# terryye/cuda_FlashAttention

Measured on AMD Instinct MI355X. Metric: FA2 fwd+bwd TFLOP/s at (B=4,H=16,N=8192,d=128); % MFMA peak, higher is better.
Workload: dtype bf16; 1 GPU; FA2 forward+backward bf16, (B=4,H=16,N=8192,d=128) per GPU, non-causal (BASELINE configs[2]); flops = 14 B H N^2 d; B=4, H=16, N=8192, d=128, parallelism=head-sharded replicas x1

## Files before the change

### cuda_flashattention_amd/csrc/fa2_bwd_bf16.hip

```cpp
#include <type_traits>

#include "fa2_regfile.h"
#include "fa2_launch.h"

namespace fa2 {

constexpr float kNoKeyRC = -1.0e30f;
constexpr float kNoKeyLq = 1.0e30f;

template <int D>
__global__ void __launch_bounds__(256) fa2_bwd_delta_kernel(const __bf16* __restrict__ dO,
                                                            const __bf16* __restrict__ O,
                                                            const float* __restrict__ L, const float* __restrict__ dL,
                                                            float* __restrict__ Dv, float* __restrict__ RC,
                                                            size_t rows, int nq, int q_hs, int q_row0, size_t rc_plane,
                                                            float inv_scale)
{
    const size_t r = ((size_t)blockIdx.x * 256 + threadIdx.x) >> 4;
    const int sub = threadIdx.x & 15;
    const size_t head = r / (size_t)nq, i = r % (size_t)nq;
    const size_t row = head * (size_t)q_hs + i;
    const size_t prow = row + (size_t)q_row0;
    float acc = 0.0f;
    if (r < rows) {
#pragma unroll
        for (int c = sub * 8; c < D; c += 128) {
            const bf16x8 a = *reinterpret_cast<const bf16x8*>(dO + row * D + c);
            const bf16x8 b = *reinterpret_cast<const bf16x8*>(O + row * D + c);
#pragma unroll
            for (int e = 0; e < 8; ++e) acc += (float)a[e] * (float)b[e];
        }
    }
#pragma unroll
    for (int off = 8; off >= 1; off >>= 1) acc += __shfl_xor(acc, off, 16);
    if (r < rows && sub == 0) {
        const float l = L[row];
        if (dL) {
            const float g = dL[row];
            acc -= l == -INFINITY ? 0.0f : g;
        }
        Dv[prow] = acc;
        RC[prow] = l == -INFINITY ? kNoKeyRC : -l * inv_scale;
        RC[rc_plane + prow] = -acc;
    }
}

__global__ void __launch_bounds__(256) fa2_bwd_dsink_kernel(const float* __restrict__ Dv, const float* __restrict__ L,
                                                            const float* __restrict__ sink, float* __restrict__ dsink,
                                                            int batch, int heads, int nq, int q_hs, int q_row0)
{
// ... 439 lines not shown
            constexpr int dt = decltype(G)::value / 4, g = decltype(G)::value % 4;
            constexpr int RK = A_DK + 16 * (kb * DT + dt) + 4 * g, RV = A_DV + 16 * (kb * DT + dt) + 4 * g;
            bf16x4 a, b;
            a[0] = (__bf16)(aread<RK>() * p.scale); a[1] = (__bf16)(aread<RK + 1>() * p.scale);
            a[2] = (__bf16)(aread<RK + 2>() * p.scale); a[3] = (__bf16)(aread<RK + 3>() * p.scale);
            b[0] = (__bf16)aread<RV>(); b[1] = (__bf16)aread<RV + 1>();
            b[2] = (__bf16)aread<RV + 2>(); b[3] = (__bf16)aread<RV + 3>();
            if (key < N) {
                *reinterpret_cast<bf16x4*>(dKk + 2 * (32 * dt + 8 * g + 4 * h)) = a;
                *reinterpret_cast<bf16x4*>(dVk + 2 * (32 * dt + 8 * g + 4 * h)) = b;
            }
        });
    });
}

template <int D, bool CAUSAL>
__global__ void __launch_bounds__(256, 1) __attribute__((amdgpu_num_vgpr(60))) fa2_bwd_dkdv_kernel(BwdArgs p)
{
    const int ncb = (p.Nk + kDkKeys - 1) / kDkKeys;
    int kvhead, cb;
    map_block(blockIdx.x, p.BH / p.kv_group, ncb, kvhead, cb);
    bwd_dkdv_impl<D, CAUSAL>(p, kvhead, cb);
}

template <int D, bool CAUSAL>
__global__ void __launch_bounds__(256, 1) __attribute__((amdgpu_num_vgpr(60))) fa2_bwd_dkdv_varlen_kernel(VarlenBwdArgs v)
{
    int kvhead, idx;
    map_block(blockIdx.x, v.a.BH / v.a.kv_group, v.n_key_items, kvhead, idx);
    const VarlenItem it = uniform_item(v.key_items, idx);
    bwd_dkdv_impl<D, CAUSAL>(bwd_varlen_view<D>(v.a, it), kvhead, it.block);
}

template <int D, bool CAUSAL>
static hipError_t launch_bwd_one(const BwdArgs& a, hipStream_t stream, const SinkGrad* sg)
{
    const size_t rows = (size_t)a.BH * a.Nq;
    hipError_t e = hipSuccess;
    if (a.phases & 1) {
        hipLaunchKernelGGL((fa2_bwd_delta_kernel<D>), dim3((unsigned)((rows * 16 + 255) / 256)), dim3(256), 0,
                           stream, (const __bf16*)a.dO, (const __bf16*)a.O, a.L, sg ? sg->dL : nullptr, a.D, a.RC, rows, a.Nq, a.q_hs,
                           a.q_row0, (size_t)a.BH * a.q_hs, 1.0f / a.scale);
        e = hipGetLastError();
        if (e != hipSuccess) return e;
        if (sg && sg->sink && (e = launch_dsink(*sg, a, a.Nq, stream)) != hipSuccess) return e;
    }
    const int nb = (a.Nq + kBwdRows - 1) / kBwdRows;
    constexpr int lds_dq = 3 * 2 * kDqKV * D * 2;
    constexpr int lds_dk = kDkKeys * D * 2 + 2 * (2 * 2 * kDkQ * D * 2 + 512);
    if (a.phases & 2) {
        e = launch_lds<fa2_bwd_dq_kernel<D, CAUSAL>>(dim3((unsigned)(nb * a.BH)), dim3(256), lds_dq, stream, a);
        if (e != hipSuccess) return e;
    }
    if (a.phases & 4) {
        const int ncb = (a.Nk + kDkKeys - 1) / kDkKeys;
        e = launch_lds<fa2_bwd_dkdv_kernel<D, CAUSAL>>(dim3((unsigned)(ncb * (a.BH / a.kv_group))), dim3(256), lds_dk, stream, a);
    }
    return e;
}

template <int D, bool CAUSAL>
static hipError_t launch_bwd_varlen_one(const VarlenBwdArgs& v, hipStream_t stream, const SinkGrad* sg)
{
    const BwdArgs& a = v.a;
    const size_t rows = (size_t)a.BH * a.q_hs;
    hipLaunchKernelGGL((fa2_bwd_delta_kernel<D>), dim3((unsigned)((rows * 16 + 255) / 256)), dim3(256), 0, stream,
                       (const __bf16*)a.dO, (const __bf16*)a.O, a.L, sg ? sg->dL : nullptr, a.D, a.RC, rows, a.q_hs, a.q_hs, 0, rows,
                       1.0f / a.scale);
    hipError_t e = hipGetLastError();
    if (e != hipSuccess) return e;
    if (sg && sg->sink && (e = launch_dsink(*sg, a, a.q_hs, stream)) != hipSuccess) return e;
    constexpr int lds_dq = 3 * 2 * kDqKV * D * 2;
    constexpr int lds_dk = kDkKeys * D * 2 + 2 * (2 * 2 * kDkQ * D * 2 + 512);
    e = launch_lds<fa2_bwd_dq_varlen_kernel<D, CAUSAL>>(dim3((unsigned)(v.n_row_items * a.BH)), dim3(256), lds_dq, stream, v);
    if (e != hipSuccess) return e;
    return launch_lds<fa2_bwd_dkdv_varlen_kernel<D, CAUSAL>>(dim3((unsigned)(v.n_key_items * (a.BH / a.kv_group))), dim3(256), lds_dk,
                                                            stream, v);
}

hipError_t launch_bwd_varlen_bf16(const VarlenBwdArgs& v, hipStream_t stream, const SinkGrad* sg)
{
    const BwdArgs& a = v.a;
    if (a.kv_group < 1 || a.BH % a.kv_group != 0 || v.n_row_items < 1 || v.n_key_items < 1 || !v.row_items || !v.key_items)
        return hipErrorInvalidValue;
    if (a.d == 128) return a.causal ? launch_bwd_varlen_one<128, true>(v, stream, sg) : launch_bwd_varlen_one<128, false>(v, stream, sg);
    if (a.d == 64) return a.causal ? launch_bwd_varlen_one<64, true>(v, stream, sg) : launch_bwd_varlen_one<64, false>(v, stream, sg);
    return hipErrorInvalidValue;
}

hipError_t launch_bwd_bf16(const BwdArgs& a, hipStream_t stream, const SinkGrad* sg)
{
    if (a.kv_group < 1 || a.BH % a.kv_group != 0) return hipErrorInvalidValue;
    if (a.d == 128) return a.causal ? launch_bwd_one<128, true>(a, stream, sg) : launch_bwd_one<128, false>(a, stream, sg);
    if (a.d == 64) return a.causal ? launch_bwd_one<64, true>(a, stream, sg) : launch_bwd_one<64, false>(a, stream, sg);
    return hipErrorInvalidValue;
}

}
```

### cuda_flashattention_amd/csrc/fa2_bwd_fused.hip

```cpp
#include <cstdlib>
#include <cstring>
#include <type_traits>

#include "fa2_regfile.h"
#include "fa2_launch.h"

namespace fa2 {

#include "fa2_bwd_fused_body.inc"

typedef __attribute__((address_space(3))) void* fused_lptr_t;

#ifndef FA2_FUSED_DSKEY
#define FA2_FUSED_DSKEY(row) (((row) >> 1) & 7)
#endif

#ifndef FA2_FUSED_DIAG
#define FA2_FUSED_DIAG 0
#endif

constexpr int kFusedRegFile = RF512;

#define FA2_FUSED_CLOBBERS "memory", "vcc", FA2_RF512
#define FA2_FUSED_OPS_128 [r0] "v"(roff[0]), [r1] "v"(roff[1]), [r2] "v"(roff[2]), [r3] "v"(roff[3]), [r4] "v"(roff[4]), [r5] "v"(roff[5]),  \
// ... 50 lines not shown
        "buffer_atomic_add_f32 v%c9, %0, %1, s12 offen offset:1024\n\tbuffer_atomic_add_f32 v%c10, %0, %1, s12 offen offset:1536\n\t"
        "buffer_atomic_add_f32 v%c11, %0, %1, s13 offen\n\tbuffer_atomic_add_f32 v%c12, %0, %1, s13 offen offset:512\n\t"
        "buffer_atomic_add_f32 v%c13, %0, %1, s13 offen offset:1024\n\tbuffer_atomic_add_f32 v%c14, %0, %1, s13 offen offset:1536\n\t"
        "buffer_atomic_add_f32 v%c15, %0, %1, s14 offen\n\tbuffer_atomic_add_f32 v%c16, %0, %1, s14 offen offset:512\n\t"
        "buffer_atomic_add_f32 v%c17, %0, %1, s14 offen offset:1024\n\tbuffer_atomic_add_f32 v%c18, %0, %1, s14 offen offset:1536\n\t"
        "s_nop 1"
        : : "v"(voff), "s"(rs), "s"(soff), "i"(DQT), "i"(DQT + 1), "i"(DQT + 2), "i"(DQT + 3), "i"(DQT + 4), "i"(DQT + 5), "i"(DQT + 6),
            "i"(DQT + 7), "i"(DQT + 8), "i"(DQT + 9), "i"(DQT + 10), "i"(DQT + 11), "i"(DQT + 12), "i"(DQT + 13), "i"(DQT + 14),
            "i"(DQT + 15)
        : "memory", "s12", "s13", "s14", "v255");
}

template <int VF, int KS, int S>
__device__ __forceinline__ void fused_load_vfrag(const char* v0, const char* v1)
{
#ifndef FA2_FUSED_KV_NT
#define FA2_FUSED_KV_NT ""
#define FA2_FUSED_KV_AUX 0
#endif
    asm volatile("global_load_dwordx4 v[%c2:%c3], %0, off offset:%c4" FA2_FUSED_KV_NT "\n\tglobal_load_dwordx4 v[%c5:%c6], %1, off offset:%c4" FA2_FUSED_KV_NT
                 : : "v"(v0), "v"(v1), "i"(VF + 4 * S), "i"(VF + 4 * S + 3), "i"(32 * S), "i"(VF + 4 * (KS + S)), "i"(VF + 4 * (KS + S) + 3)
                 : "memory", "v255");
}

template <int DQT>
__device__ __forceinline__ void fused_dq_zero()
{
    static_for<16>([&](auto R) { vset<kFusedRegFile, CL_TOP, DQT + decltype(R)::value>(0u); });
}

constexpr int kCtlTicket = 0, kCtlNextHead = 32 * 16, kCtlError = 32 * 17, kCtlHeadmap = 32 * 18;
constexpr int kHmPad = 16;
constexpr int kSpinLimit = FA2_FUSED_SPIN_LIMIT;

struct FusedArgs {
    BwdArgs b;
    float* dQacc;
    int* ctl;
    int npad;
    const float* rc;
    int fault;
};

#ifdef FA2_TEST_HOOKS
static int g_hook_fault = 0, g_hook_grid = 0, g_hook_last_grid = 0;
extern "C" void fa2_test_set_fused_hooks(int fault, int grid) { g_hook_fault = fault; g_hook_grid = grid; }
extern "C" int fa2_test_last_fused_grid(void) { return g_hook_last_grid; }
#define FA2_HOOK_NOTE_GRID(n) (g_hook_last_grid = (n))
#else
constexpr int g_hook_fault = 0, g_hook_grid = 0;
#define FA2_HOOK_NOTE_GRID(n) ((void)0)
#endif

__device__ __forceinline__ int fused_ctl_ints(int BH, int ncb) { return kCtlHeadmap + 16 * (BH + kHmPad) + 9 * BH * ncb; }

__device__ __forceinline__ int fused_load_sc1(const int* p)
{
    int v;
    asm volatile("global_load_dword %0, %1, off sc1\n\ts_waitcnt vmcnt(0)" : "=v"(v) : "v"(p) : "memory");
    return v;
}
__device__ __forceinline__ void fused_seen_set(int v)
{
    asm volatile("v_mov_b32 v39, %0" : : "s"(v) : "v39");
}

__device__ __forceinline__ int fused_lane_id() { return (int)__builtin_amdgcn_mbcnt_hi(~0u, __builtin_amdgcn_mbcnt_lo(~0u, 0u)); }
template <int OFF>
__device__ __forceinline__ int fused_mail_read(uint32_t lds_addr)
{
    int v;
    asm volatile("v_mov_b32 %0, %1\n\tds_read_b32 %0, %0 offset:%c2\n\ts_waitcnt lgkmcnt(0)" : "=&v"(v) : "s"(lds_addr), "i"(OFF) : "memory");
    return __builtin_amdgcn_readfirstlane(v);
}

__device__ __forceinline__ void fused_store_flag(int* p, int v)
{
    asm volatile("global_store_dword %0, %1, off" : : "v"(p), "v"(v) : "memory");
}

__device__ __forceinline__ bool fused_spin_over(int* ctl, int spins)
{
    if (spins > kSpinLimit) {
        atomicExch(ctl + kCtlError, 1);
        return true;
    }
    return (spins & 1023) == 0 && fused_load_sc1(ctl + kCtlError) != 0;
}

template <bool CHAIN, bool CAUSAL, bool RAGGED = false, bool RECT = false, int HD = 128>
__global__ void __launch_bounds__(256, 1) __attribute__((amdgpu_num_vgpr(39))) fa2_bwd_fused_kernel(FusedArgs fp)
{
    static_assert(CHAIN || !RAGGED, "the atomics form has no ragged variant");
    static_assert(!RECT || (CHAIN && !CAUSAL && !RAGGED), "rectangular blocks: chained, unmasked, aligned");
    static_assert(HD == 128 || (HD == 64 && CHAIN && !RECT), "head_dim 64: chained, square");
    extern __shared__ __attribute__((aligned(16))) char smem[];
    const BwdArgs& p = fp.b;
    constexpr int D = HD, ROWB = 2 * D, KS = D / 16, DT = D / 32;
    constexpr int DQW = 128;
    constexpr int TROWS = 32;
    constexpr bool W = D == 128;
    constexpr int QRING = W ? FA2_FUSED_QRING : FA2_FUSED64_QRING, BUFB = W ? FA2_FUSED_BUFB : FA2_FUSED64_BUFB,
                  DSB = W ? FA2_FUSED_DSB : FA2_FUSED64_DSB, LDSB = W ? FA2_FUSED_LDS : FA2_FUSED64_LDS;
    constexpr int CPR = D / 8, RPI = 64 / CPR, NINS = TROWS / RPI;
    constexpr int VF = W ? FA2_FUSED_VF : FA2_FUSED64_VF, DQT = W ? FA2_FUSED_DQT : FA2_FUSED64_DQT,
                  ROFFK = W ? FA2_FUSED_ROFFK : FA2_FUSED64_ROFFK, DSWR = W ? FA2_FUSED_DSWR : FA2_FUSED64_DSWR,
                  DSRD = W ? FA2_FUSED_DSRD : FA2_FUSED64_DSRD, KT = W ? FA2_FUSED_KT : FA2_FUSED64_KT;
    constexpr int VMW = CHAIN ? (W ? 4 : 2) : 63;
    int* const mail = reinterpret_cast<int*>(smem + LDSB);
    const uint32_t mail_addr = __builtin_amdgcn_readfirstlane((uint32_t)(uintptr_t)smem) + LDSB;

    const int tid = threadIdx.x;
    const int lane = tid & 63;
    const int wave = __builtin_amdgcn_readfirstlane(tid >> 6);
    const int ki = lane & 31;
    const int h = lane >> 5;
    const int N = p.Nk;
    const int NP = RAGGED ? fp.npad : N;
    const int NQ = RECT ? p.Nq : N;
    const int NPQ = RECT ? NQ : NP;
    const int QHS = RECT ? p.q_hs : N, KHS = RECT ? p.k_hs : N;
    const int QR0 = RECT ? p.q_row0 : 0;
    const int ncb = NP / 256;
    const int ntiles = NPQ / TROWS;
    const int niter = ((ntiles + 1 + 5) / 6) * 6;
    const float c2 = p.scale * kLog2e;
    const size_t rc_plane = (size_t)p.BH * (RECT ? QHS : NP);

    const uint32_t lbase = (uint32_t)(uintptr_t)smem;
    const int trq = (lane & 15) >> 2, trp = lane & 3, trcb = (lane >> 4) & 1;
    uint32_t roff[KS], toff[2 * DT];
#pragma unroll
    for (int s = 0; s < KS; ++s) roff[s] = lbase + QRING + lds_off<D>(ki, 2 * s + h);
#pragma unroll
// ... 128 lines not shown
                const int soff = (t * TROWS + piece * RPI) * ROWB;
                __builtin_amdgcn_raw_ptr_buffer_load_lds(which ? g_rsrc : q_rsrc, (fused_lptr_t)(b + which * (TROWS * ROWB) + piece * 1024),
                                                         16, doff, soff, 0, 0);
            }
            if (wave < 2 && fused_lane_id() < 32)
                __builtin_amdgcn_raw_ptr_buffer_load_lds(rc_rsrc, (fused_lptr_t)(b + 2 * TROWS * ROWB + wave * 128), 4, rcoff, t * TROWS * 4, 0, 0);
        };
        const int n_u = CAUSAL ? ntiles - 8 * cb : ntiles;
        const int niter_u = CAUSAL ? ((n_u + 1 + 5) / 6) * 6 : niter;
        const bool ragged_unit = RAGGED && !CAUSAL && cb == ncb - 1;
        const int first_masked = CAUSAL ? ((n_u - 8) / 6) * 6 : (ragged_unit ? 0 : niter_u);
        auto tl = [&](int u) { return CAUSAL ? ntiles - 1 - u : u; };
        stage(tl(0), 0);
#ifdef FA2_FUSED_PREFILL
        stage(tl(1), 1);
        stage(tl(2), 2);
#endif
        fused_dq_zero<DQT>();
        asm volatile("s_waitcnt vmcnt(0)" ::: "memory");
        __syncthreads();
        if constexpr (W) asm volatile(FA2_FUSED_PRO : : FA2_FUSED_OPS_128, [vm] "i"(VMW) : FA2_FUSED_CLOBBERS);
        else asm volatile(FA2_FUSED64_PRO : : FA2_FUSED_OPS_64, [vm] "i"(VMW) : FA2_FUSED_CLOBBERS);

        const auto dq_rsrc = __builtin_amdgcn_make_buffer_rsrc((void*)(fp.dQacc + (size_t)head * NPQ * DQW), 0, NPQ * DQW * 4, 0x00020000);
        int* const mine = prog_base + head * ncb + cb;
        const int* const prev = mine - 1;
        const int prev_off = (int)((prev - fp.ctl) * 4);
        const int mine_off = (int)((mine - fp.ctl) * 4);
        if constexpr (CHAIN) fused_seen_set(0);
        int err = err0;
#ifdef FA2_FUSED_STATS
        int st_steps = 0, st_polls = 0, st_cycles = 0;
        const uint64_t u0 = __builtin_readcyclecounter();
#endif

        const auto null_rsrc = __builtin_amdgcn_make_buffer_rsrc((void*)fp.dQacc, 0, 0, 0x00020000);
        const bool hp_unit = cb > 0;
        const auto lrs_unit = hp_unit && !(FA2_FUSED_DIAG & 2) ? dq_rsrc : null_rsrc;
        auto step = [&](auto BUF, auto PAR, auto MASKED, auto FAST_, int t) {
            constexpr int buf = decltype(BUF)::value, par = decltype(PAR)::value;
            constexpr bool masked = decltype(MASKED)::value;
            constexpr bool FAST = decltype(FAST_)::value;
            if constexpr (CHAIN && FAST) {
                FusedStep f;
                f.drs = dq_rsrc;
                f.lrs = lrs_unit;
                f.dso = (uint32_t)(tl(t - 1) * TROWS * DQW * 4);
                f.lso = (uint32_t)(tl(t) * TROWS * DQW * 4);
                f.qrs = q_rsrc; f.grs = g_rsrc; f.rcrs = rc_rsrc; f.ctl = ctl_rsrc;
                f.qso = (uint32_t)(tl(t + 1) * TROWS * ROWB + wave * 1024);
                f.rcso = (uint32_t)(tl(t + 1) * TROWS * 4);
                f.pvo = (uint32_t)prev_off; f.mso = (uint32_t)mine_off;
                f.need = (hp_unit && !err && !(FA2_FUSED_DIAG & 1)) ? t + 1 : (int)0x80000000;
                f.pval = t;
#ifdef FA2_TEST_HOOKS
                if (fp.fault && cb == 1) f.pval = 0;
#endif
                fused_cbody<D, buf, par, VMW, false>(roff, toff, rcv, c2, dqv, (uint32_t)doff, (uint32_t)rcoff, lbase + QRING + wave * 1024,
                                                  lbase + QRING + wave * 128, wave, f, err, 0, 0);
            } else if constexpr (CHAIN) {
                FusedStep f;
                const bool live = t >= 1 && t <= n_u;
                const bool more = t + 1 < n_u;
                const bool has_prev = t < n_u && cb > 0;
                f.drs = live ? dq_rsrc : null_rsrc;
                f.lrs = has_prev && !(FA2_FUSED_DIAG & 2) ? dq_rsrc : null_rsrc;
// ... 37 lines not shown
                fused_dq_zero<DQT>();
            }
        };
        auto six = [&](auto MASKED, auto FAST_, int t) {
            step(std::integral_constant<int, 0>{}, std::integral_constant<int, 0>{}, MASKED, FAST_, t);
            step(std::integral_constant<int, 1>{}, std::integral_constant<int, 1>{}, MASKED, FAST_, t + 1);
            step(std::integral_constant<int, 2>{}, std::integral_constant<int, 0>{}, MASKED, FAST_, t + 2);
            step(std::integral_constant<int, 0>{}, std::integral_constant<int, 1>{}, MASKED, FAST_, t + 3);
            step(std::integral_constant<int, 1>{}, std::integral_constant<int, 0>{}, MASKED, FAST_, t + 4);
            step(std::integral_constant<int, 2>{}, std::integral_constant<int, 1>{}, MASKED, FAST_, t + 5);
        };
        const int fast_end = CHAIN ? n_u - 2 : -1;
        {
            const int plain_end = first_masked;
            int t = 0;
            asm volatile("" : "+s"(t));
            if (t < plain_end) { six(std::false_type{}, std::false_type{}, t); t += 6; }
#pragma unroll 1
            for (; t + 5 <= fast_end && t < plain_end; t += 6) six(std::false_type{}, std::true_type{}, t);
#pragma unroll 1
            for (; t < plain_end; t += 6) six(std::false_type{}, std::false_type{}, t);
            if constexpr (CHAIN && (CAUSAL || RAGGED)) {
#pragma unroll 1
                for (; t < niter_u; t += 6) six(std::true_type{}, std::false_type{}, t);
            }
        }
        asm volatile("s_waitcnt vmcnt(0) lgkmcnt(0)" ::: "memory");
        if constexpr (CHAIN)
            if (err && !err0 && wave == 0 && fused_lane_id() == 0) atomicExch(fp.ctl + kCtlError, 1);
#ifdef FA2_FUSED_STATS
        const uint64_t s_loop = __builtin_readcyclecounter();
#endif
        next_unit_loads();

        mfma_acc_settle();
        const int lane_ep = (int)__builtin_amdgcn_mbcnt_hi(~0u, __builtin_amdgcn_mbcnt_lo(~0u, 0u));
        const int ki_ep = lane_ep & 31, h_ep = lane_ep >> 5;
        static_for<2>([&](auto KB) {
            constexpr int kb = decltype(KB)::value;
            const int key = kw0 + 32 * kb + ki_ep;
            const size_t slab_k = RECT ? (size_t)head * KHS * ROWB : slab;
            char* const dKb = (char*)p.dK + slab_k;
            char* const dVb = (char*)p.dV + slab_k;
            const uint32_t koff = (uint32_t)key * ROWB + 16u * h_ep;
            char* dKk = dKb + koff;
            char* dVk = dVb + koff;
            static_for<2 * DT>([&](auto G) {
                constexpr int dt = decltype(G)::value / 2, gp = decltype(G)::value % 2;
                constexpr int RK = 16 * (kb * DT + dt) + 8 * gp, RV = 32 * DT + RK;
                auto pack4 = [&](float a, float b, float c, float d, float sc) {
                    bf16x4 v;
                    v[0] = (__bf16)(a * sc); v[1] = (__bf16)(b * sc); v[2] = (__bf16)(c * sc); v[3] = (__bf16)(d * sc);
                    return __builtin_bit_cast(u32x2, v);
                };
                auto emit = [&](u32x2 x, u32x2 y, char* dst) {
                    const auto s0 = __builtin_amdgcn_permlane32_swap(x[0], y[0], false, false);
                    const auto s1 = __builtin_amdgcn_permlane32_swap(x[1], y[1], false, false);
                    const u32x4 o = {s0[0], s1[0], s0[1], s1[1]};
#ifdef FA2_FUSED_ST_NT
                    if (!RAGGED || key < N) __builtin_nontemporal_store(o, reinterpret_cast<u32x4*>(dst + 2 * (32 * dt + 16 * gp)));
#else
                    if (!RAGGED || key < N) *reinterpret_cast<u32x4*>(dst + 2 * (32 * dt + 16 * gp)) = o;
#endif
                };
                emit(pack4(aread<RK>(), aread<RK + 1>(), aread<RK + 2>(), aread<RK + 3>(), p.scale),
                     pack4(aread<RK + 4>(), aread<RK + 5>(), aread<RK + 6>(), aread<RK + 7>(), p.scale), dKk);
                emit(pack4(aread<RV>(), aread<RV + 1>(), aread<RV + 2>(), aread<RV + 3>(), 1.0f),
                     pack4(aread<RV + 4>(), aread<RV + 5>(), aread<RV + 6>(), aread<RV + 7>(), 1.0f), dVk);
            });
        });
#ifdef FA2_FUSED_STATS
        if (CHAIN && wave == 0 && fused_lane_id() == 0) {
            atomicAdd(fp.ctl + kCtlError + 1, st_steps);
            atomicAdd(fp.ctl + kCtlError + 2, st_polls);
            atomicAdd((unsigned long long*)(fp.ctl + kCtlError + 4), (unsigned long long)st_cycles);
            atomicAdd((unsigned long long*)(fp.ctl + kCtlError + 6), (unsigned long long)(__builtin_readcyclecounter() - u0));
            int* rec = prog_base + p.BH * ncb + 8 * (head * ncb + cb);
            rec[0] = xcc; rec[1] = st_cycles; rec[2] = (int)(u0 - s_pull); rec[3] = (int)(__builtin_readcyclecounter() - s_loop);
            *(unsigned long long*)(rec + 4) = u0; *(unsigned long long*)(rec + 6) = __builtin_readcyclecounter();
        }
#endif
        if constexpr (!CHAIN) break;
    }
}

__global__ void __launch_bounds__(256) fa2_bwd_fused_dq_out_kernel(const float* __restrict__ acc, __bf16* __restrict__ dQ, size_t n8, float scale,
                                                                    const int* __restrict__ err)
{
    const float poison = (err && *err) ? __builtin_nanf("") : 0.0f;
    const size_t stride = (size_t)gridDim.x * 256;
    for (size_t i = (size_t)blockIdx.x * 256 + threadIdx.x; i < n8; i += stride) {
        const f32x4 a = reinterpret_cast<const f32x4*>(acc)[2 * i], b = reinterpret_cast<const f32x4*>(acc)[2 * i + 1];
        bf16x8 o;
#pragma unroll
        for (int e = 0; e < 4; ++e) { o[e] = (__bf16)(a[e] * scale + poison); o[4 + e] = (__bf16)(b[e] * scale + poison); }
        reinterpret_cast<bf16x8*>(dQ)[i] = o;
    }
}

__global__ void __launch_bounds__(256) fa2_bwd_fused_dq_out_chain_kernel(const float* __restrict__ acc, __bf16* __restrict__ dQ, size_t n4, float scale,
                                                                          const int* __restrict__ err, int N, int NP, int qhs)
{
    const float poison = *err ? __builtin_nanf("") : 0.0f;
    const size_t stride = (size_t)gridDim.x * 256;
    const size_t tiles = (size_t)(NP / 32);
    for (size_t i = (size_t)blockIdx.x * 256 + threadIdx.x; i < n4; i += stride) {
        const f32x4 a = reinterpret_cast<const f32x4*>(acc)[i];
        const int lane = (int)(i & 63), g = (int)((i >> 6) & 3), wave = (int)((i >> 8) & 3);
        const size_t tg = i >> 10, head = tg / tiles;
        const int row = (int)(tg % tiles) * 32 + 8 * g + 4 * (lane >> 5);
        __bf16* o = dQ + (head * (size_t)qhs + row) * 128 + 32 * wave + (lane & 31);
#pragma unroll
        for (int e = 0; e < 4; ++e)
            if (row + e < N) o[(size_t)e * 128] = (__bf16)(a[e] * scale + poison);
    }
}

__global__ void __launch_bounds__(256) fa2_bwd_fused_dq_out_chain64_kernel(const float* __restrict__ acc, __bf16* __restrict__ dQ, size_t n4h, float scale,
                                                                            const int* __restrict__ err, int N, int NP)
{
    const float poison = *err ? __builtin_nanf("") : 0.0f;
    const size_t stride = (size_t)gridDim.x * 256;
    const size_t tiles = (size_t)(NP / 32);
    for (size_t i = (size_t)blockIdx.x * 256 + threadIdx.x; i < n4h; i += stride) {
        const int lane = (int)(i & 63), g = (int)((i >> 6) & 3), cbk = (int)((i >> 8) & 1);
        const size_t tg = i >> 9, head = tg / tiles;
        const size_t slot = ((tg * 4 + cbk) * 4 + g) * 64 + lane;
        const f32x4 a = reinterpret_cast<const f32x4*>(acc)[slot], b = reinterpret_cast<const f32x4*>(acc)[slot + 2 * 4 * 64];
        const int row = (int)(tg % tiles) * 32 + 8 * g + 4 * (lane >> 5);
        __bf16* o = dQ + (head * (size_t)N + row) * 64 + 32 * cbk + (lane & 31);
#pragma unroll
        for (int e = 0; e < 4; ++e)
            if (row + e < N) o[(size_t)e * 64] = (__bf16)((a[e] + b[e]) * scale + poison);
    }
}

__global__ void __launch_bounds__(256) fa2_bwd_fused_dkdv_out_kernel(const bf16x8* __restrict__ pK, const bf16x8* __restrict__ pV,
                                                                      bf16x8* __restrict__ dK, bf16x8* __restrict__ dV, size_t n8, size_t nkv, int G)
{
    const size_t stride = (size_t)gridDim.x * 256;
    for (size_t i = (size_t)blockIdx.x * 256 + threadIdx.x; i < 2 * nkv * n8; i += stride) {
        const bool isv = i >= nkv * n8;
        const size_t o = isv ? i - nkv * n8 : i, kvh = o / n8, r = o % n8;
        const bf16x8* src = (isv ? pV : pK) + kvh * (size_t)G * n8 + r;
        float s[8] = {};
        for (int g = 0; g < G; ++g) {
            const bf16x8 x = src[(size_t)g * n8];
// ... 43 lines not shown
hipError_t bwd_fused_clear_error(int* ctl, hipStream_t stream)
{
    return launch_fill_f32(reinterpret_cast<float*>(ctl + kCtlError), 1, 0.0f, stream);
}

size_t bwd_fused_kvpart_bytes(int BH, int N, int d) { return (size_t)2 * BH * N * d * 2; }
size_t bwd_fused_ctl_bytes(int BH, int N) { return (size_t)(kCtlHeadmap + 16 * (BH + kHmPad) + 9 * BH * ((N + 255) / 256)) * sizeof(int); }

template <int HD>
static hipError_t launch_chained_square(bool causal, bool ragged, dim3 grid, int lds, hipStream_t stream, const FusedArgs& fa)
{
    if (causal)
        return ragged ? launch_lds<fa2_bwd_fused_kernel<true, true, true, false, HD>>(grid, dim3(256), lds, stream, fa)
                      : launch_lds<fa2_bwd_fused_kernel<true, true, false, false, HD>>(grid, dim3(256), lds, stream, fa);
    return ragged ? launch_lds<fa2_bwd_fused_kernel<true, false, true, false, HD>>(grid, dim3(256), lds, stream, fa)
                  : launch_lds<fa2_bwd_fused_kernel<true, false, false, false, HD>>(grid, dim3(256), lds, stream, fa);
}

hipError_t launch_bwd_fused_bf16(const BwdArgs& a, float* dQacc, int* ctl, int mode, hipStream_t stream, float* rcpad, void* kvpart,
                                 const SinkGrad* sg)
{
    const int npad = (a.Nk + 255) / 256 * 256;
    const bool ragged = npad != a.Nk;
    const bool rect = a.Nq != a.Nk || a.q_hs != a.Nq || a.k_hs != a.Nk || a.q_row0 != 0;
    if ((a.d != 128 && a.d != 64) || a.Nk < 1 || a.Nq < 1) return hipErrorInvalidValue;
    if (a.d == 64 && (mode != 1 || rect)) return hipErrorInvalidValue;
    if (rect && (mode != 1 || a.causal || ragged || a.Nq % 32 != 0 || a.q_row0 < 0 || a.q_hs < a.q_row0 + a.Nq || a.k_hs < a.Nk))
        return hipErrorInvalidValue;
    if (ragged && (mode != 1 || !rcpad)) return hipErrorInvalidValue;
    const bool grouped = a.kv_group > 1;
    if (a.kv_group < 1 || a.BH % a.kv_group != 0 || (grouped && (mode != 1 || rect || !kvpart))) return hipErrorInvalidValue;
    if (a.causal && (mode != 1 || a.causal_shift != 0)) return hipErrorInvalidValue;
    hipError_t e = hipSuccess;
    if (a.phases & 1) {
        BwdArgs d = a;
        d.phases = 1;
        e = launch_bwd_bf16(d, stream, sg);
        if (e != hipSuccess) return e;
    }
    if (!(a.phases & 8)) return hipSuccess;
    const size_t elems = (size_t)a.BH * (rect ? a.Nq : npad) * 128;
    const int units = a.BH * (npad / 256);
    if (ragged) {
        const size_t n = (size_t)2 * a.BH * npad;
        hipLaunchKernelGGL(fa2_bwd_fused_rcpad_kernel, dim3((unsigned)((n + 255) / 256)), dim3(256), 0, stream, (const float*)a.RC, rcpad,
                           a.BH, a.Nk, npad);
        e = hipGetLastError();
        if (e != hipSuccess) return e;
    }
    FusedArgs fa{a, dQacc, ctl, npad, ragged ? (const float*)rcpad : (const float*)a.RC, g_hook_fault};
    const size_t part_elems = (size_t)a.BH * a.Nk * a.d;
    if (grouped) {
        fa.b.dK = kvpart;
        fa.b.dV = (__bf16*)kvpart + part_elems;
    }
    const int lds = (a.d == 64 ? FA2_FUSED64_LDS : FA2_FUSED_LDS) + 16;
    if (mode == 0) {
        e = launch_fill_f32(dQacc, elems, 0.0f, stream);
        if (e != hipSuccess) return e;
        e = bwd_fused_clear_error(ctl, stream);
        if (e != hipSuccess) return e;
        e = launch_lds<fa2_bwd_fused_kernel<false, false>>(dim3((unsigned)units), dim3(256), lds, stream, fa);
    } else {
        static int cus[64] = {};
        int dev = 0;
        e = hipGetDevice(&dev);
        if (e != hipSuccess) return e;
        if (dev < 0 || dev >= 64) return hipErrorInvalidDevice;
        if (!cus[dev]) {
            e = hipDeviceGetAttribute(&cus[dev], hipDeviceAttributeMultiprocessorCount, dev);
            if (e != hipSuccess) return e;
        }
        e = launch_fill_f32(reinterpret_cast<float*>(ctl), bwd_fused_ctl_bytes(a.BH, a.Nk) / sizeof(float), 0.0f, stream);
        if (e != hipSuccess) return e;
        int avail = cus[dev] - (a.reserve_cus > 0 ? a.reserve_cus : 0);
        if (avail < 1) avail = 1;
        int wgs = units < avail ? units : avail;
        if (g_hook_grid >= 1 && g_hook_grid < wgs) wgs = g_hook_grid;
        FA2_HOOK_NOTE_GRID(wgs);
        const dim3 grid((unsigned)wgs);
        if (rect)
            e = launch_lds<fa2_bwd_fused_kernel<true, false, false, true>>(grid, dim3(256), lds, stream, fa);
        else
            e = a.d == 64 ? launch_chained_square<64>(a.causal, ragged, grid, lds, stream, fa)
                          : launch_chained_square<128>(a.causal, ragged, grid, lds, stream, fa);
    }
    if (e != hipSuccess) return e;
    if (mode == 0)
        hipLaunchKernelGGL(fa2_bwd_fused_dq_out_kernel, dim3(2048), dim3(256), 0, stream, dQacc, (__bf16*)a.dQ, elems / 8, a.scale,
                           (const int*)nullptr);
    else if (a.d == 64)
        hipLaunchKernelGGL(fa2_bwd_fused_dq_out_chain64_kernel, dim3(4096), dim3(256), 0, stream, dQacc, (__bf16*)a.dQ, elems / 8, a.scale,
                           ctl + kCtlError, a.Nk, npad);
    else
        hipLaunchKernelGGL(fa2_bwd_fused_dq_out_chain_kernel, dim3(4096), dim3(256), 0, stream, dQacc, (__bf16*)a.dQ, elems / 4, a.scale,
                           ctl + kCtlError, rect ? a.Nq : a.Nk, rect ? a.Nq : npad, rect ? a.q_hs : a.Nk);
    e = hipGetLastError();
    if (e != hipSuccess || !grouped) return e;
    hipLaunchKernelGGL(fa2_bwd_fused_dkdv_out_kernel, dim3(4096), dim3(256), 0, stream, (const bf16x8*)fa.b.dK, (const bf16x8*)fa.b.dV,
                       (bf16x8*)a.dK, (bf16x8*)a.dV, (size_t)a.Nk * a.d / 8, (size_t)(a.BH / a.kv_group), a.kv_group);
    return hipGetLastError();
}

}
```

### cuda_flashattention_amd/csrc/fa2_launch.h

```cpp
#pragma once
#include <hip/hip_runtime.h>
#include <stddef.h>

namespace fa2 {

struct FwdArgs {
    const void* Q;
    const void* K;
    const void* V;
    void* O;
    float* L;
    float* Oacc;
    float* M;
    int BH, Nq, Nk, d;
    float scale;
    int causal;
    int causal_shift;
    int resume;
    int finalize;
    int q_hs, k_hs;
    int kv_group;
    const float* sink;
    int sink_heads;
};
// ... 48 lines not shown
struct FwdFp8Args {
    const void* Q; const void* K; const void* V;
    void* Vt;
    float* kn;
    void* O;
    float* L;
    int BH, N, Npad, d;
    float scale;
    int causal;
    float o_scale;
};
hipError_t launch_fwd_fp8(const FwdFp8Args& a, hipStream_t stream);

struct BwdArgs {
    const void* Q; const void* K; const void* V; const void* O; const void* dO;
    const float* L;
    void* dQ; void* dK; void* dV;
    float* D;
    float* RC;
    int BH, Nq, Nk, d;
    int q_hs, k_hs;
    int q_row0;
    float scale;
    int causal;
    int causal_shift;
    int phases;
    int reserve_cus;
    int kv_group;
};

struct SinkGrad { const float* sink; float* dsink; int heads; const float* dL = nullptr; };

hipError_t launch_bwd_bf16(const BwdArgs& a, hipStream_t stream, const SinkGrad* sg = nullptr);
struct VarlenBwdArgs {
    BwdArgs a;
    const VarlenItem* row_items; const VarlenItem* key_items;
    int n_row_items, n_key_items;
};
hipError_t launch_bwd_varlen_bf16(const VarlenBwdArgs& v, hipStream_t stream, const SinkGrad* sg = nullptr);
size_t bwd_fused_ctl_bytes(int BH, int N);
size_t bwd_fused_kvpart_bytes(int BH, int N, int d);
hipError_t launch_bwd_fused_bf16(const BwdArgs& a, float* dQacc, int* ctl, int mode, hipStream_t stream, float* rcpad = nullptr,
                                 void* kvpart = nullptr, const SinkGrad* sg = nullptr);
bool bwd_fused_device_ok(const char** why);
hipError_t bwd_fused_read_error(const int* ctl, int* err, hipStream_t stream);
hipError_t bwd_fused_clear_error(int* ctl, hipStream_t stream);

struct F32Args {
    const float* Q; const float* K; const float* V; float* O; float* L;
    const float* dO; float* dQ; float* dK; float* dV; float* D;
    int BH, N, d;
    float scale;
    int causal;
    int phases;
    int Nk;
    float* M;
    int resume, finalize;
};
hipError_t launch_fwd_f32(const F32Args& a, hipStream_t stream);
hipError_t launch_bwd_f32(const F32Args& a, hipStream_t stream);

template <auto K, typename A>
inline hipError_t launch_lds(dim3 grid, dim3 block, int lds, hipStream_t stream, const A& arg)
{
    static bool done[64] = {};
    int dev = 0;
// ... 23 lines not shown
```

Measured before the change: 1298 TFLOP/s.

## Convert dQ tail inside fused bwd kernel and fold ctl zeroing into delta kernel

```diff
diff --git a/cuda_flashattention_amd/csrc/fa2_bwd_bf16.hip b/cuda_flashattention_amd/csrc/fa2_bwd_bf16.hip
--- a/cuda_flashattention_amd/csrc/fa2_bwd_bf16.hip
+++ b/cuda_flashattention_amd/csrc/fa2_bwd_bf16.hip
@@ -14,8 +14,9 @@
                                                             const float* __restrict__ L, const float* __restrict__ dL,
                                                             float* __restrict__ Dv, float* __restrict__ RC,
                                                             size_t rows, int nq, int q_hs, int q_row0, size_t rc_plane,
-                                                            float inv_scale)
-{
+                                                            float inv_scale, int* __restrict__ zero, unsigned zero_n)
+{
+    for (size_t z = (size_t)blockIdx.x * 256 + threadIdx.x; z < zero_n; z += (size_t)gridDim.x * 256) zero[z] = 0;
     const size_t r = ((size_t)blockIdx.x * 256 + threadIdx.x) >> 4;
     const int sub = threadIdx.x & 15;
     const size_t head = r / (size_t)nq, i = r % (size_t)nq;
@@ -521,16 +522,22 @@
     bwd_dkdv_impl<D, CAUSAL>(bwd_varlen_view<D>(v.a, it), kvhead, it.block);
 }
 
+template <int D>
+static hipError_t launch_delta(const BwdArgs& a, hipStream_t stream, const SinkGrad* sg, int* zero, unsigned zero_n)
+{
+    const size_t rows = (size_t)a.BH * a.Nq;
+    hipLaunchKernelGGL((fa2_bwd_delta_kernel<D>), dim3((unsigned)((rows * 16 + 255) / 256)), dim3(256), 0,
+                       stream, (const __bf16*)a.dO, (const __bf16*)a.O, a.L, sg ? sg->dL : nullptr, a.D, a.RC, rows, a.Nq, a.q_hs,
+                       a.q_row0, (size_t)a.BH * a.q_hs, 1.0f / a.scale, zero, zero_n);
+    return hipGetLastError();
+}
+
 template <int D, bool CAUSAL>
 static hipError_t launch_bwd_one(const BwdArgs& a, hipStream_t stream, const SinkGrad* sg)
 {
-    const size_t rows = (size_t)a.BH * a.Nq;
     hipError_t e = hipSuccess;
     if (a.phases & 1) {
-        hipLaunchKernelGGL((fa2_bwd_delta_kernel<D>), dim3((unsigned)((rows * 16 + 255) / 256)), dim3(256), 0,
-                           stream, (const __bf16*)a.dO, (const __bf16*)a.O, a.L, sg ? sg->dL : nullptr, a.D, a.RC, rows, a.Nq, a.q_hs,
-                           a.q_row0, (size_t)a.BH * a.q_hs, 1.0f / a.scale);
-        e = hipGetLastError();
+        e = launch_delta<D>(a, stream, sg, nullptr, 0);
         if (e != hipSuccess) return e;
         if (sg && sg->sink && (e = launch_dsink(*sg, a, a.Nq, stream)) != hipSuccess) return e;
     }
@@ -555,7 +562,7 @@
     const size_t rows = (size_t)a.BH * a.q_hs;
     hipLaunchKernelGGL((fa2_bwd_delta_kernel<D>), dim3((unsigned)((rows * 16 + 255) / 256)), dim3(256), 0, stream,
                        (const __bf16*)a.dO, (const __bf16*)a.O, a.L, sg ? sg->dL : nullptr, a.D, a.RC, rows, a.q_hs, a.q_hs, 0, rows,
-                       1.0f / a.scale);
+                       1.0f / a.scale, (int*)nullptr, 0u);
     hipError_t e = hipGetLastError();
     if (e != hipSuccess) return e;
     if (sg && sg->sink && (e = launch_dsink(*sg, a, a.q_hs, stream)) != hipSuccess) return e;
@@ -585,4 +592,12 @@
     return hipErrorInvalidValue;
 }
 
-}
+hipError_t launch_bwd_delta_zero_bf16(const BwdArgs& a, int* zero, size_t zero_n, hipStream_t stream)
+{
+    if (a.kv_group < 1 || a.BH % a.kv_group != 0 || !zero || zero_n > 0xffffffffu) return hipErrorInvalidValue;
+    if (a.d == 128) return launch_delta<128>(a, stream, nullptr, zero, (unsigned)zero_n);
+    if (a.d == 64) return launch_delta<64>(a, stream, nullptr, zero, (unsigned)zero_n);
+    return hipErrorInvalidValue;
+}
+
+}
diff --git a/cuda_flashattention_amd/csrc/fa2_bwd_fused.hip b/cuda_flashattention_amd/csrc/fa2_bwd_fused.hip
--- a/cuda_flashattention_amd/csrc/fa2_bwd_fused.hip
+++ b/cuda_flashattention_amd/csrc/fa2_bwd_fused.hip
@@ -106,6 +106,18 @@
 constexpr int kCtlTicket = 0, kCtlNextHead = 32 * 16, kCtlError = 32 * 17, kCtlHeadmap = 32 * 18;
 constexpr int kHmPad = 16;
 constexpr int kSpinLimit = FA2_FUSED_SPIN_LIMIT;
+#ifndef FA2_FUSED_TAIL_TILES
+#define FA2_FUSED_TAIL_TILES 8
+#endif
+#ifndef FA2_FUSED_TAIL_LD_AUX
+#define FA2_FUSED_TAIL_LD_AUX 16
+#endif
+constexpr int kTailTiles = FA2_FUSED_TAIL_TILES;
+#ifdef FA2_FUSED_STATS
+constexpr bool kTailBuilt = false;
+#else
+constexpr bool kTailBuilt = true;
+#endif
 
 struct FusedArgs {
     BwdArgs b;
@@ -114,6 +126,7 @@
     int npad;
     const float* rc;
     int fault;
+    int tail;
 };
 
 #ifdef FA2_TEST_HOOKS
@@ -121,9 +134,29 @@
 extern "C" void fa2_test_set_fused_hooks(int fault, int grid) { g_hook_fault = fault; g_hook_grid = grid; }
 extern "C" int fa2_test_last_fused_grid(void) { return g_hook_last_grid; }
 #define FA2_HOOK_NOTE_GRID(n) (g_hook_last_grid = (n))
+static int g_hook_tail = 1, g_hook_tail_heads = 0, g_hook_tail_cph = 0;
+static const int* g_hook_tail_claim = nullptr;
+static hipStream_t g_hook_tail_stream = nullptr;
+extern "C" void fa2_test_set_fused_tail(int on) { g_hook_tail = on; }
+extern "C" int fa2_test_fused_tail_claimed(void)
+{
+    if (!g_hook_tail_claim || g_hook_tail_heads < 1 || hipStreamSynchronize(g_hook_tail_stream) != hipSuccess) return -1;
+    int* host = (int*)malloc(sizeof(int) * (size_t)g_hook_tail_heads);
+    if (!host) return -1;
+    int sum = -1;
+    if (hipMemcpy(host, g_hook_tail_claim, sizeof(int) * (size_t)g_hook_tail_heads, hipMemcpyDeviceToHost) == hipSuccess) {
+        sum = 0;
+        for (int i = 0; i < g_hook_tail_heads; ++i) sum += host[i] < g_hook_tail_cph ? host[i] : g_hook_tail_cph;
+    }
+    free(host);
+    return sum;
+}
+#define FA2_HOOK_NOTE_TAIL(claim, heads, cph, stream) \
+    (g_hook_tail_claim = (claim), g_hook_tail_heads = (heads), g_hook_tail_cph = (cph), g_hook_tail_stream = (stream))
 #else
 constexpr int g_hook_fault = 0, g_hook_grid = 0;
 #define FA2_HOOK_NOTE_GRID(n) ((void)0)
+#define FA2_HOOK_NOTE_TAIL(claim, heads, cph, stream) ((void)(cph))
 #endif
 
 __device__ __forceinline__ int fused_ctl_ints(int BH, int ncb) { return kCtlHeadmap + 16 * (BH + kHmPad) + 9 * BH * ncb; }
@@ -161,6 +194,8 @@
     }
     return (spins & 1023) == 0 && fused_load_sc1(ctl + kCtlError) != 0;
 }
+
+__device__ __forceinline__ __bf16 fused_dq_round(float a, float scale, float poison) { return (__bf16)(a * scale + poison); }
 
 template <bool CHAIN, bool CAUSAL, bool RAGGED = false, bool RECT = false, int HD = 128>
 __global__ void __launch_bounds__(256, 1) __attribute__((amdgpu_num_vgpr(39))) fa2_bwd_fused_kernel(FusedArgs fp)
@@ -174,6 +209,7 @@
     constexpr int DQW = 128;
     constexpr int TROWS = 32;
     constexpr bool W = D == 128;
+    constexpr bool TAIL = kTailBuilt && CHAIN && !CAUSAL && !RAGGED && !RECT && W;
     constexpr int QRING = W ? FA2_FUSED_QRING : FA2_FUSED64_QRING, BUFB = W ? FA2_FUSED_BUFB : FA2_FUSED64_BUFB,
                   DSB = W ? FA2_FUSED_DSB : FA2_FUSED64_DSB, LDSB = W ? FA2_FUSED_LDS : FA2_FUSED64_LDS;
     constexpr int CPR = D / 8, RPI = 64 / CPR, NINS = TROWS / RPI;
@@ -368,6 +404,7 @@
 #ifdef FA2_FUSED_STATS
         int st_steps = 0, st_polls = 0, st_cycles = 0;
         const uint64_t u0 = __builtin_readcyclecounter();
+        const uint64_t u0_rt = __builtin_amdgcn_s_memrealtime();
 #endif
 
         const auto null_rsrc = __builtin_amdgcn_make_buffer_rsrc((void*)fp.dQacc, 0, 0, 0x00020000);
@@ -471,6 +508,8 @@
         const uint64_t s_loop = __builtin_readcyclecounter();
 #endif
         next_unit_loads();
+        if constexpr (TAIL)
+            if (cb == ncb - 1 && !err && wave == 0 && fused_lane_id() == 0) fused_store_flag(prog_base + p.BH * ncb + head, 1);
 
         mfma_acc_settle();
         const int lane_ep = (int)__builtin_amdgcn_mbcnt_hi(~0u, __builtin_amdgcn_mbcnt_lo(~0u, 0u));
@@ -516,10 +555,73 @@
             atomicAdd((unsigned long long*)(fp.ctl + kCtlError + 6), (unsigned long long)(__builtin_readcyclecounter() - u0));
             int* rec = prog_base + p.BH * ncb + 8 * (head * ncb + cb);
             rec[0] = xcc; rec[1] = st_cycles; rec[2] = (int)(u0 - s_pull); rec[3] = (int)(__builtin_readcyclecounter() - s_loop);
-            *(unsigned long long*)(rec + 4) = u0; *(unsigned long long*)(rec + 6) = __builtin_readcyclecounter();
+            *(unsigned long long*)(rec + 4) = u0_rt; *(unsigned long long*)(rec + 6) = __builtin_amdgcn_s_memrealtime();
         }
 #endif
         if constexpr (!CHAIN) break;
+    }
+
+    if constexpr (TAIL) {
+        static_assert(!TAIL || kTailTiles * 16384 <= LDSB, "a chunk is staged below the mailbox");
+        if (!fp.tail) return;
+        int* const tail_base = prog_base + p.BH * ncb;
+        const int nchunks = ntiles / kTailTiles;
+        const int lane_t = fused_lane_id();
+        const uint32_t dma_voff = (uint32_t)(16 * (8 * (lane_t & 7) + (lane_t >> 3)));
+        const int e_t = lane_t & 3, a_t = (lane_t >> 2) & 7, b_t = lane_t >> 5;
+        const int* const hm = fp.ctl + kCtlHeadmap + xcc * (p.BH + kHmPad);
+        __syncthreads();
+        int k = 0;
+        for (;;) {
+            if (wave == 0 && lane_t == 0) {
+                int hd = -1, c = -1;
+                if (fused_load_sc1(fp.ctl + kCtlError) == 0) {
+                    while (k < p.BH + kHmPad) {
+                        const int v = fused_load_sc1(hm + k);
+                        if (v <= 0 || v > p.BH) { k = p.BH + kHmPad; break; }
+                        if (fused_load_sc1(tail_base + v - 1) == 1) {
+                            c = atomicAdd(tail_base + p.BH + v - 1, 1);
+                            if (c >= 0 && c < nchunks) { hd = v - 1; break; }
+                        }
+                        ++k;
+                    }
+                }
+                mail[0] = hd;
+                mail[3] = c;
+            }
+            __syncthreads();
+            const int hd = fused_mail_read<0>(mail_addr);
+            const int c = fused_mail_read<12>(mail_addr);
+            if (hd < 0 || hd >= p.BH || c < 0 || c >= nchunks) break;
+            const auto acc_rsrc = __builtin_amdgcn_make_buffer_rsrc((void*)(fp.dQacc + (size_t)hd * N * DQW), 0, N * DQW * 4, 0x00020000);
+            __bf16* const dq_head = (__bf16*)p.dQ + (size_t)hd * N * D;
+            const uint32_t soff = (uint32_t)c * (kTailTiles * 16384);
+#pragma unroll
+            for (int j = wave; j < kTailTiles * 16; j += 4)
+                __builtin_amdgcn_raw_ptr_buffer_load_lds(acc_rsrc, (fused_lptr_t)(smem + j * 1024), 16, dma_voff, soff + j * 1024, 0,
+                                                         FA2_FUSED_TAIL_LD_AUX);
+            asm volatile("s_waitcnt vmcnt(0)" ::: "memory");
+            __syncthreads();
+#pragma unroll 2
+            for (int it = 0; it < kTailTiles * 2; ++it) {
+                const int q = it * 4 + wave;
+                const int w = 2 * (q & 1) + b_t, g = (q >> 1) & 3, t = q >> 3;
+                const char* src = smem + ((t * 4 + w) * 4 + g) * 1024 + a_t * 16 + e_t * 4;
+                float x[8];
+#pragma unroll
+                for (int i = 0; i < 8; ++i) x[i] = *reinterpret_cast<const float*>(src + i * 128);
+                bf16x8 o;
+#pragma unroll
+                for (int i = 0; i < 8; ++i) o[i] = fused_dq_round(x[i], p.scale, 0.0f);
+                const int row = (c * kTailTiles + t) * TROWS + 8 * g + 4 * (a_t >> 2) + e_t;
+                u32x4* dst = reinterpret_cast<u32x4*>(dq_head + (size_t)row * D + 32 * w + 8 * (a_t & 3));
+#ifdef FA2_FUSED_TAIL_ST_NT
+                __builtin_nontemporal_store(__builtin_bit_cast(u32x4, o), dst);
+#else
+                *dst = __builtin_bit_cast(u32x4, o);
+#endif
+            }
+        }
     }
 }
 
@@ -537,21 +639,28 @@
     }
 }
 
-__global__ void __launch_bounds__(256) fa2_bwd_fused_dq_out_chain_kernel(const float* __restrict__ acc, __bf16* __restrict__ dQ, size_t n4, float scale,
-                                                                          const int* __restrict__ err, int N, int NP, int qhs)
-{
-    const float poison = *err ? __builtin_nanf("") : 0.0f;
-    const size_t stride = (size_t)gridDim.x * 256;
-    const size_t tiles = (size_t)(NP / 32);
-    for (size_t i = (size_t)blockIdx.x * 256 + threadIdx.x; i < n4; i += stride) {
-        const f32x4 a = reinterpret_cast<const f32x4*>(acc)[i];
-        const int lane = (int)(i & 63), g = (int)((i >> 6) & 3), wave = (int)((i >> 8) & 3);
-        const size_t tg = i >> 10, head = tg / tiles;
-        const int row = (int)(tg % tiles) * 32 + 8 * g + 4 * (lane >> 5);
-        __bf16* o = dQ + (head * (size_t)qhs + row) * 128 + 32 * wave + (lane & 31);
-#pragma unroll
-        for (int e = 0; e < 4; ++e)
-            if (row + e < N) o[(size_t)e * 128] = (__bf16)(a[e] * scale + poison);
+__global__ void __launch_bounds__(256) fa2_bwd_fused_dq_out_chain_kernel(const float* __restrict__ acc, __bf16* __restrict__ dQ, int heads, float scale,
+                                                                          const int* __restrict__ err, int N, int NP, int qhs,
+                                                                          const int* __restrict__ claim)
+{
+    const bool bad = *err != 0;
+    const float poison = bad ? __builtin_nanf("") : 0.0f;
+    const int tiles = NP / 32;
+    const size_t items = (size_t)heads * tiles;
+    for (size_t item = blockIdx.x; item < items; item += gridDim.x) {
+        const int head = (int)(item / tiles), tile = (int)(item % tiles);
+        if (claim && !bad && tile / kTailTiles < claim[head]) continue;
+#pragma unroll
+        for (int k = 0; k < 4; ++k) {
+            const size_t i = (item << 10) + 256 * k + threadIdx.x;
+            const f32x4 a = reinterpret_cast<const f32x4*>(acc)[i];
+            const int lane = (int)(i & 63), g = (int)((i >> 6) & 3), wave = (int)((i >> 8) & 3);
+            const int row = tile * 32 + 8 * g + 4 * (lane >> 5);
+            __bf16* o = dQ + ((size_t)head * qhs + row) * 128 + 32 * wave + (lane & 31);
+#pragma unroll
+            for (int e = 0; e < 4; ++e)
+                if (row + e < N) o[(size_t)e * 128] = fused_dq_round(a[e], scale, poison);
+        }
     }
 }
 
@@ -661,7 +770,11 @@
     if (a.kv_group < 1 || a.BH % a.kv_group != 0 || (grouped && (mode != 1 || rect || !kvpart))) return hipErrorInvalidValue;
     if (a.causal && (mode != 1 || a.causal_shift != 0)) return hipErrorInvalidValue;
     hipError_t e = hipSuccess;
-    if (a.phases & 1) {
+    const bool ctl_by_delta = mode == 1 && (a.phases & 9) == 9 && !sg;
+    if (ctl_by_delta) {
+        e = launch_bwd_delta_zero_bf16(a, ctl, bwd_fused_ctl_bytes(a.BH, a.Nk) / sizeof(int), stream);
+        if (e != hipSuccess) return e;
+    } else if (a.phases & 1) {
         BwdArgs d = a;
         d.phases = 1;
         e = launch_bwd_bf16(d, stream, sg);
@@ -677,7 +790,7 @@
         e = hipGetLastError();
         if (e != hipSuccess) return e;
     }
-    FusedArgs fa{a, dQacc, ctl, npad, ragged ? (const float*)rcpad : (const float*)a.RC, g_hook_fault};
+    FusedArgs fa{a, dQacc, ctl, npad, ragged ? (const float*)rcpad : (const float*)a.RC, g_hook_fault, 0};
     const size_t part_elems = (size_t)a.BH * a.Nk * a.d;
     if (grouped) {
         fa.b.dK = kvpart;
@@ -700,13 +813,20 @@
             e = hipDeviceGetAttribute(&cus[dev], hipDeviceAttributeMultiprocessorCount, dev);
             if (e != hipSuccess) return e;
         }
-        e = launch_fill_f32(reinterpret_cast<float*>(ctl), bwd_fused_ctl_bytes(a.BH, a.Nk) / sizeof(float), 0.0f, stream);
-        if (e != hipSuccess) return e;
+        if (!ctl_by_delta) {
+            e = launch_fill_f32(reinterpret_cast<float*>(ctl), bwd_fused_ctl_bytes(a.BH, a.Nk) / sizeof(float), 0.0f, stream);
+            if (e != hipSuccess) return e;
+        }
         int avail = cus[dev] - (a.reserve_cus > 0 ? a.reserve_cus : 0);
         if (avail < 1) avail = 1;
         int wgs = units < avail ? units : avail;
         if (g_hook_grid >= 1 && g_hook_grid < wgs) wgs = g_hook_grid;
         FA2_HOOK_NOTE_GRID(wgs);
+#ifdef FA2_TEST_HOOKS
+        fa.tail = g_hook_tail;
+#else
+        fa.tail = (long long)units >= 8LL * wgs;
+#endif
         const dim3 grid((unsigned)wgs);
         if (rect)
             e = launch_lds<fa2_bwd_fused_kernel<true, false, false, true>>(grid, dim3(256), lds, stream, fa);
@@ -715,15 +835,20 @@
                           : launch_chained_square<128>(a.causal, ragged, grid, lds, stream, fa);
     }
     if (e != hipSuccess) return e;
+    const int tiles = (rect ? a.Nq : npad) / 32, cph = (tiles + kTailTiles - 1) / kTailTiles;
+    const int* claim = kTailBuilt && mode == 1 ? ctl + kCtlHeadmap + 16 * (a.BH + kHmPad) + units + a.BH : nullptr;
+    FA2_HOOK_NOTE_TAIL(claim, a.BH, cph, stream);
     if (mode == 0)
         hipLaunchKernelGGL(fa2_bwd_fused_dq_out_kernel, dim3(2048), dim3(256), 0, stream, dQacc, (__bf16*)a.dQ, elems / 8, a.scale,
                            (const int*)nullptr);
     else if (a.d == 64)
         hipLaunchKernelGGL(fa2_bwd_fused_dq_out_chain64_kernel, dim3(4096), dim3(256), 0, stream, dQacc, (__bf16*)a.dQ, elems / 8, a.scale,
                            ctl + kCtlError, a.Nk, npad);
-    else
-        hipLaunchKernelGGL(fa2_bwd_fused_dq_out_chain_kernel, dim3(4096), dim3(256), 0, stream, dQacc, (__bf16*)a.dQ, elems / 4, a.scale,
-                           ctl + kCtlError, rect ? a.Nq : a.Nk, rect ? a.Nq : npad, rect ? a.q_hs : a.Nk);
+    else {
+        const long long items = (long long)a.BH * tiles;
+        hipLaunchKernelGGL(fa2_bwd_fused_dq_out_chain_kernel, dim3((unsigned)(items < 4096 ? items : 4096)), dim3(256), 0, stream, dQacc,
+                           (__bf16*)a.dQ, a.BH, a.scale, ctl + kCtlError, rect ? a.Nq : a.Nk, rect ? a.Nq : npad, rect ? a.q_hs : a.Nk, claim);
+    }
     e = hipGetLastError();
     if (e != hipSuccess || !grouped) return e;
     hipLaunchKernelGGL(fa2_bwd_fused_dkdv_out_kernel, dim3(4096), dim3(256), 0, stream, (const bf16x8*)fa.b.dK, (const bf16x8*)fa.b.dV,
diff --git a/cuda_flashattention_amd/csrc/fa2_launch.h b/cuda_flashattention_amd/csrc/fa2_launch.h
--- a/cuda_flashattention_amd/csrc/fa2_launch.h
+++ b/cuda_flashattention_amd/csrc/fa2_launch.h
@@ -104,6 +104,7 @@
 struct SinkGrad { const float* sink; float* dsink; int heads; const float* dL = nullptr; };
 
 hipError_t launch_bwd_bf16(const BwdArgs& a, hipStream_t stream, const SinkGrad* sg = nullptr);
+hipError_t launch_bwd_delta_zero_bf16(const BwdArgs& a, int* zero, size_t zero_n, hipStream_t stream);
 struct VarlenBwdArgs {
     BwdArgs a;
     const VarlenItem* row_items; const VarlenItem* key_items;
```

After: 1298 TFLOP/s. About the same (-0.0%).
